# abajcsy/legged_games_gym

Measured on AMD Instinct MI355X. Metric: env-steps/sec (whole node), ANYmal-C flat 4096 envs/GPU, higher is better.
Workload: dtype f32; 1 GPU; anymal_c_flat, 4096 envs/GPU, plane, actuator-net torques, self-collision ON (asset.self_collisions = 0), random-init policy [48, 128, 64, 32, 12] rollout (act = mu + sigma*eps), fixed command (0.5,0,0), obs noise + friction/mass randomisation + pushes on; envs_per_gpu=4096, decimation=4, parallelism=env-sharded x1, state_finite=True, policy=MFMA actor inside k_step (v_mfma_f32_16x16x4_f32, 4 waves)

## Files before the change

legged_games_gym_amd/csrc/lg_device.h:

```cpp
#pragma once
#include <hip/hip_runtime.h>
#include <stdint.h>
#include "../../include/legged_hip.h"

#define LG_DEV __device__ __forceinline__

namespace lg {

struct V3 { float x, y, z; };
LG_DEV V3 v3(float x, float y, float z) { V3 r; r.x = x; r.y = y; r.z = z; return r; }
LG_DEV V3 operator+(V3 a, V3 b) { return v3(a.x + b.x, a.y + b.y, a.z + b.z); }
LG_DEV V3 operator-(V3 a, V3 b) { return v3(a.x - b.x, a.y - b.y, a.z - b.z); }
LG_DEV V3 operator*(V3 a, float s) { return v3(a.x * s, a.y * s, a.z * s); }
LG_DEV float dot(V3 a, V3 b) { return a.x * b.x + a.y * b.y + a.z * b.z; }
LG_DEV V3 cross(V3 a, V3 b) { return v3(a.y * b.z - a.z * b.y, a.z * b.x - a.x * b.z, a.x * b.y - a.y * b.x); }
struct M3 { float m[9]; };
LG_DEV V3 mul(const M3 &R, V3 a) {
    return v3(R.m[0] * a.x + R.m[1] * a.y + R.m[2] * a.z, R.m[3] * a.x + R.m[4] * a.y + R.m[5] * a.z,
              R.m[6] * a.x + R.m[7] * a.y + R.m[8] * a.z);
}
LG_DEV M3 mul(const M3 &A, const M3 &B) {
    M3 C;
#pragma unroll
    for (int i = 0; i < 3; i++)
#pragma unroll
        for (int j = 0; j < 3; j++) C.m[3 * i + j] = A.m[3 * i] * B.m[j] + A.m[3 * i + 1] * B.m[3 + j] + A.m[3 * i + 2] * B.m[6 + j];
    return C;
}
LG_DEV V3 symv(const float *S, V3 a) {
    return v3(S[0] * a.x + S[1] * a.y + S[2] * a.z, S[1] * a.x + S[3] * a.y + S[4] * a.z, S[2] * a.x + S[4] * a.y + S[5] * a.z);
}
struct S6 { V3 w, v; };
LG_DEV S6 operator+(S6 a, S6 b) { S6 r; r.w = a.w + b.w; r.v = a.v + b.v; return r; }
LG_DEV S6 operator*(S6 a, float k) { S6 r; r.w = a.w * k; r.v = a.v * k; return r; }
LG_DEV float dot(S6 a, S6 b) { return dot(a.w, b.w) + dot(a.v, b.v); }

struct AI { float A[6], H[9], M[6]; };
LG_DEV void ai_add(AI &a, const AI &b) {
#pragma unroll
    for (int i = 0; i < 6; i++) { a.A[i] += b.A[i]; a.M[i] += b.M[i]; }
#pragma unroll
    for (int i = 0; i < 9; i++) a.H[i] += b.H[i];
}
LG_DEV void ai_add_point(AI &I, float m, V3 c) {
    float cc = dot(c, c);
    I.A[0] += m * (cc - c.x * c.x); I.A[1] -= m * c.x * c.y; I.A[2] -= m * c.x * c.z;
    I.A[3] += m * (cc - c.y * c.y); I.A[4] -= m * c.y * c.z; I.A[5] += m * (cc - c.z * c.z);
    I.H[1] -= m * c.z; I.H[2] += m * c.y; I.H[3] += m * c.z; I.H[5] -= m * c.x; I.H[6] -= m * c.y; I.H[7] += m * c.x;
    I.M[0] += m; I.M[3] += m; I.M[5] += m;
}
LG_DEV void ai_add_rank1(AI &I, float k, V3 gw, V3 gv) {
    float w[3] = {gw.x, gw.y, gw.z}, v[3] = {gv.x, gv.y, gv.z};
    int t = 0;
#pragma unroll
    for (int i = 0; i < 3; i++)
#pragma unroll
        for (int j = i; j < 3; j++, t++) { I.A[t] += k * w[i] * w[j]; I.M[t] += k * v[i] * v[j]; }
#pragma unroll
    for (int i = 0; i < 3; i++)
#pragma unroll
        for (int j = 0; j < 3; j++) I.H[3 * i + j] += k * w[i] * v[j];
}
LG_DEV S6 ai_mul(const AI &I, S6 s) {
    S6 r;
    M3 H; for (int i = 0; i < 9; i++) H.m[i] = I.H[i];
    r.w = symv(I.A, s.w) + mul(H, s.v);
    r.v = v3(I.H[0] * s.w.x + I.H[3] * s.w.y + I.H[6] * s.w.z, I.H[1] * s.w.x + I.H[4] * s.w.y + I.H[7] * s.w.z,
             I.H[2] * s.w.x + I.H[5] * s.w.y + I.H[8] * s.w.z) + symv(I.M, s.v);
    return r;
}

LG_DEV S6 ai_mul_w(const AI &I, V3 w) {
    S6 r;
    r.w = symv(I.A, w);
    r.v = v3(I.H[0] * w.x + I.H[3] * w.y + I.H[6] * w.z, I.H[1] * w.x + I.H[4] * w.y + I.H[7] * w.z,
             I.H[2] * w.x + I.H[5] * w.y + I.H[8] * w.z);
    return r;
}
LG_DEV void ai_shift(AI &I, S6 &p, V3 d) {
    const int ix[3][3] = {{0, 1, 2}, {1, 3, 4}, {2, 4, 5}};
    float T[9];
#pragma unroll
    for (int j = 0; j < 3; j++) {
        V3 x = cross(d, v3(I.M[ix[0][j]], I.M[ix[1][j]], I.M[ix[2][j]]));
        T[j] = I.H[j] + x.x; T[3 + j] = I.H[3 + j] + x.y; T[6 + j] = I.H[6 + j] + x.z;
    }
    V3 dxh[3], txd[3];
#pragma unroll
    for (int j = 0; j < 3; j++) dxh[j] = cross(d, v3(I.H[3 * j], I.H[3 * j + 1], I.H[3 * j + 2]));
#pragma unroll
    for (int i = 0; i < 3; i++) txd[i] = cross(v3(T[3 * i], T[3 * i + 1], T[3 * i + 2]), d);
    float A2[6];
#pragma unroll
    for (int i = 0; i < 3; i++)
#pragma unroll
        for (int j = i; j < 3; j++) {
            float a = (i == 0) ? dxh[j].x : (i == 1) ? dxh[j].y : dxh[j].z;
            float b = (j == 0) ? txd[i].x : (j == 1) ? txd[i].y : txd[i].z;
            A2[ix[i][j]] = I.A[ix[i][j]] + a - b;
        }
#pragma unroll
    for (int i = 0; i < 6; i++) I.A[i] = A2[i];
#pragma unroll
// ... 187 lines not shown
```

legged_games_gym_amd/csrc/lg_kernels.hip:

```cpp
#include <hip/hip_runtime.h>
#include <math.h>
#include <stdio.h>
#include <string.h>
#include <new>

#define LG_POLICY_BLOCKS_ONLY
#include "lg_host.h"

using namespace lg;

#define LG_BLOCK 64
#define LG_JS 40
#define LG_PASSES 2
#define LG_STEP_WAVES 4

struct AnymalTraits {
    static constexpr int K = 4, L = 3, NREP = 4, NPT = 5;
    static constexpr int pt_joint(int i) { return i < 2 ? 1 : 2; }
    static constexpr int pt_rep(int i) { return i < 2 ? 1 : (i < 4 ? 2 : 3); }
    static constexpr int FOOT_REP = 3;
    static constexpr int NCAP = 3, NGRP = 2;
    static constexpr int cap_p0(int c) { return 2 * c; }
    static constexpr int cap_p1(int c) { return c < 2 ? 2 * c + 1 : 4; }
    static constexpr int cap_grp(int c) { return c == 0 ? 0 : 1; }
// ... 315 lines not shown
        float vn = dot(c.n, c.vc);
        V3 vt = c.vc - c.n * vn;
        V3 f = c.n * (P.contact_stiffness * c.depth - kn * vn) - vt * c.bt + c.fs;
        ai_add_point(IA, dt * c.bt, c.r);
        ai_add_rank1(IA, dt * (kn - c.bt), cross(c.r, c.n), c.n);
        pA.w = pA.w - cross(c.r, f);
        pA.v = pA.v - f;
    }
}
template <bool HF>
LG_DEV void contact_evaluate(Contact &c, const lg_params &P, float kn, float mu, S6 acc, bool more = true) {
    if constexpr (!HF) {
        if (c.on) {
            V3 v1 = c.vc + (acc.v + cross(acc.w, c.r)) * P.sim_dt;
            float fn = plane_normal_force(P, kn, c.depth, v1.z);
            if (fn <= 0.0f) { c.on = false; c.f = v3(0, 0, 0); }
            else {
                c.f = plane_force(c, v1, fn);
                if (!more) return;
                float vtm = plane_slip_speed(v1), cone = mu * fn;
                if (c.bt * vtm > cone) { const float s = -cone / vtm; c.fs = v3(v1.x * s, v1.y * s, 0.0f); c.bt = 0.0f; }
                else if (c.bt > 0.0f) c.bt = fminf(P.friction_damping, cone / fmaxf(vtm, P.stick_velocity));
            }
        }
        return;
    }
    if (c.on) {
        V3 v1 = c.vc + (acc.v + cross(acc.w, c.r)) * P.sim_dt;
        float vn = dot(c.n, v1);
        V3 vt = v1 - c.n * vn;
        float fn = P.contact_stiffness * c.depth - kn * vn;
        if (fn <= 0.0f) { c.on = false; c.f = v3(0, 0, 0); }
        else {
            c.f = c.n * fn - vt * c.bt + c.fs;
            if (!more) return;
            float vtm = sqrtf(dot(vt, vt)), cone = mu * fn;
            if (c.bt * vtm > cone) { c.fs = vt * (-cone / vtm); c.bt = 0.0f; }
            else if (c.bt > 0.0f) c.bt = fminf(P.friction_damping, cone / fmaxf(vtm, P.stick_velocity));
        }
    }
}

LG_DEV float motor_torque(float tau, float qd, float vlim) {
    if (vlim <= 0.0f || tau * qd <= 0.0f) return tau;
    float s = (vlim - fabsf(qd)) / (0.1f * vlim);
    return tau * fminf(fmaxf(s, 0.0f), 1.0f);
}
LG_DEV V3 clamp_norm(V3 a, float lim) {
    float n2 = dot(a, a);
    if (!(n2 <= lim * lim)) { float k = (n2 > 0.0f && n2 < INFINITY) ? lim * __builtin_amdgcn_rsqf(n2) : 0.0f; return a * k; }
    return a;
}

LG_DEV void body_terms(V3 grav, float m, V3 com_l, const float *Il, const M3 &R, V3 w, V3 v, AI &I0, S6 &p0) {
    V3 c = mul(R, com_l);
    M3 Ilf; Ilf.m[0] = Il[0]; Ilf.m[1] = Il[1]; Ilf.m[2] = Il[2]; Ilf.m[3] = Il[1]; Ilf.m[4] = Il[3]; Ilf.m[5] = Il[4];
    Ilf.m[6] = Il[2]; Ilf.m[7] = Il[4]; Ilf.m[8] = Il[5];
    M3 Rt;
#pragma unroll
    for (int i = 0; i < 3; i++)
#pragma unroll
        for (int j2 = 0; j2 < 3; j2++) Rt.m[3 * i + j2] = R.m[3 * j2 + i];
    M3 Ic = mul(mul(R, Ilf), Rt);
#pragma unroll
    for (int i = 0; i < 9; i++) I0.H[i] = 0.0f;
#pragma unroll
    for (int i = 0; i < 6; i++) I0.M[i] = 0.0f;
    I0.A[0] = Ic.m[0]; I0.A[1] = Ic.m[1]; I0.A[2] = Ic.m[2]; I0.A[3] = Ic.m[4]; I0.A[4] = Ic.m[5]; I0.A[5] = Ic.m[8];
    ai_add_point(I0, m, c);
    V3 l = (v + cross(w, c)) * m;
    V3 n = mul(Ic, w) + cross(c, l);
    V3 fg = grav * m;
    p0.w = (cross(w, n) + cross(v, l)) - cross(c, fg);
    p0.v = cross(w, l) - fg;
}
struct FkOut { M3 R; V3 db, ax, w, v; };
LG_DEV FkOut fk_joint(const float *tj, const M3 &Rpar, V3 wpar, V3 vpar, float q, float qd) {
    FkOut o;
    o.db = mul(Rpar, v3(tj[J_POS], tj[J_POS + 1], tj[J_POS + 2]));
    M3 Rfix;
#pragma unroll
    for (int i = 0; i < 9; i++) Rfix.m[i] = tj[J_ROT + i];
    const M3 Rz = mul(Rpar, Rfix);
    o.ax = v3(Rz.m[0], Rz.m[3], Rz.m[6]);
    float sn, cs;
    __sincosf(q, &sn, &cs);
#pragma unroll
    for (int r = 0; r < 3; r++) {
        o.R.m[3 * r] = Rz.m[3 * r];
        o.R.m[3 * r + 1] = cs * Rz.m[3 * r + 1] + sn * Rz.m[3 * r + 2];
        o.R.m[3 * r + 2] = cs * Rz.m[3 * r + 2] - sn * Rz.m[3 * r + 1];
    }
    o.w = wpar + o.ax * qd;
    o.v = vpar + cross(wpar, o.db);
    return o;
}
#define LG_BT_QUADS 7
LG_DEV void bt_store(float4 (*dst)[LG_BLOCK], int lane, const AI &I, const S6 &p) {
    dst[0][lane] = make_float4(I.A[0], I.A[1], I.A[2], I.A[3]); dst[1][lane] = make_float4(I.A[4], I.A[5], I.H[0], I.H[1]);
    dst[2][lane] = make_float4(I.H[2], I.H[3], I.H[4], I.H[5]); dst[3][lane] = make_float4(I.H[6], I.H[7], I.H[8], I.M[0]);
    dst[4][lane] = make_float4(I.M[1], I.M[2], I.M[3], I.M[4]); dst[5][lane] = make_float4(I.M[5], p.w.x, p.w.y, p.w.z);
    dst[6][lane] = make_float4(p.v.x, p.v.y, p.v.z, 0.0f);
}
LG_DEV void bt_load(const float4 (*src)[LG_BLOCK], int lane, AI &I, S6 &p) {
    float4 a = src[0][lane], b = src[1][lane], c = src[2][lane], d = src[3][lane], e = src[4][lane], f = src[5][lane], g = src[6][lane];
    I.A[0] = a.x; I.A[1] = a.y; I.A[2] = a.z; I.A[3] = a.w; I.A[4] = b.x; I.A[5] = b.y; I.H[0] = b.z; I.H[1] = b.w;
    I.H[2] = c.x; I.H[3] = c.y; I.H[4] = c.z; I.H[5] = c.w; I.H[6] = d.x; I.H[7] = d.y; I.H[8] = d.z; I.M[0] = d.w;
    I.M[1] = e.x; I.M[2] = e.y; I.M[3] = e.z; I.M[4] = e.w; I.M[5] = f.x; p.w = v3(f.y, f.z, f.w); p.v = v3(g.x, g.y, g.z);
}

#define LG_SC_REC 4
template <class T> struct SelfLds {
    float4 pos[T::NPT][LG_BLOCK];
    float4 vel[T::NPT][LG_BLOCK];
    float4 grp[T::NGRP][LG_BLOCK];
    float4 basepose[5][LG_BLOCK];
    float4 rec[T::K][T::NGRP][LG_SC_REC][LG_BLOCK];
    alignas(16) int ready[LG_STEP_WAVES];
    float4 base_pts[LG_MAX_BASE_POINTS];
};
LG_DEV V3 xyz(float4 a) { return v3(a.x, a.y, a.z); }
template <bool SA, bool SB> LG_DEV void seg_seg_closest(V3 a0, V3 a1, V3 b0, V3 b1, float &s, float &t) {
    const float eps = 1e-12f;
    V3 d1 = a1 - a0, d2 = b1 - b0, r = a0 - b0;
    float a = SA ? 0.0f : dot(d1, d1), e = SB ? 0.0f : dot(d2, d2), f = SB ? 0.0f : dot(d2, r);
    if ((SA || a <= eps) && (SB || e <= eps)) { s = 0.0f; t = 0.0f; }
    else if (SA || a <= eps) { s = 0.0f; t = fminf(fmaxf(f / e, 0.0f), 1.0f); }
    else {
        float c = dot(d1, r);
        if (SB || e <= eps) { t = 0.0f; s = fminf(fmaxf(-c / a, 0.0f), 1.0f); }
        else {
            float b = dot(d1, d2), denom = a * e - b * b;
            s = (denom > eps) ? fminf(fmaxf((b * f - c * e) / denom, 0.0f), 1.0f) : 0.0f;
            t = (b * s + f) / e;
            if (t < 0.0f) { t = 0.0f; s = fminf(fmaxf(-c / a, 0.0f), 1.0f); }
            else if (t > 1.0f) { t = 1.0f; s = fminf(fmaxf((b - c) / a, 0.0f), 1.0f); }
        }
    }
}
struct SelfHit { V3 n, pa, pb; float depth, f0; };
template <bool SA, bool SB, class Vel>
LG_DEV bool capsule_contact(const lg_params &P, float kn, V3 a0, V3 a1, float ra, V3 b0, V3 b1, float rb, Vel vel, SelfHit &h) {
    float s, t;
    seg_seg_closest<SA, SB>(a0, a1, b0, b1, s, t);
    V3 ca = a0 + (a1 - a0) * s, cb = b0 + (b1 - b0) * t, diff = ca - cb;
    float dist = sqrtf(dot(diff, diff));
    float d = ra + rb - dist;
    if (!(d > -P.contact_margin)) return false;
    V3 va0, va1, vb0, vb1;
    vel(va0, va1, vb0, vb1);
    h.n = diff * (1.0f / fmaxf(dist, 1e-9f));
    V3 va = va0 + (va1 - va0) * s, vb = vb0 + (vb1 - vb0) * t;
    float f = P.contact_stiffness * d - kn * dot(h.n, va - vb);
    if (!(d > 0.0f || f > 0.0f)) return false;
    h.depth = d; h.f0 = fmaxf(f, 0.0f); h.pa = ca - h.n * ra; h.pb = cb + h.n * rb;
    return true;
}
template <class T>
LG_DEV void self_detect(const KArgs &A, const float *lds_tab, int ln, int m, SelfLds<T> &sc) {
    constexpr int K = T::K, NCAP = T::NCAP, NGRP = T::NGRP;
    const lg_params &P = A.P;
// ... 47 lines not shown
#pragma unroll
    for (int ga = 0; ga < NGRP; ga++) {
        SelfHit best; best.depth = -1e30f; best.f0 = 0.0f; best.n = best.pa = best.pb = v3(0, 0, 0);
        float best_mB = 1.0f; int best_i = 0;
        const unsigned gbits = ((1u << NGRP) - 1u) << (ga * NGRP);
        if (any && __builtin_amdgcn_ballot_w64((cand & gbits) != 0) != 0) {
#pragma unroll 1
            for (int i = T::grp_cap_lo(ga); i < T::grp_cap_hi(ga); i++) {
                const int ip0 = T::cap_p0(i), ip1 = T::cap_p1(i);
                const float4 pa0 = sc.pos[ip0][ln], pa1 = sc.pos[ip1][ln];
                const bool sa = ip0 == ip1;
                const int nother = m == 0 ? nbc : NCAP;
#pragma unroll 1
                for (int j = 0; j < nother; j++) {
                    const unsigned bit = 1u << (ga * NGRP + (m == 0 ? 0 : T::cap_grp(j)));
                    if (__builtin_amdgcn_ballot_w64((cand & bit) != 0) == 0) continue;
                    SelfHit h; bool hit = false; float mB;
                    if (m == 0) {
                        const V3 e0 = base_end(j, 0), e1 = base_end(j, 1);
                        auto vel = [&](V3 &va0, V3 &va1, V3 &vb0, V3 &vb1) {
                            va0 = xyz(sc.vel[ip0][ln]); va1 = xyz(sc.vel[ip1][ln]); vb0 = v0 + cross(w0, e0); vb1 = v0 + cross(w0, e1);
                        };
                        mB = A.base.mass_robot;
                        if (cand & bit) hit = sa ? capsule_contact<true, false>(P, kn, xyz(pa0), xyz(pa1), pa0.w, e0, e1, sc.base_pts[2 * j].w, vel, h)
                                                 : capsule_contact<false, false>(P, kn, xyz(pa0), xyz(pa1), pa0.w, e0, e1, sc.base_pts[2 * j].w, vel, h);
                    } else {
                        const int jp0 = T::cap_p0(j), jp1 = T::cap_p1(j);
                        const float4 pb0 = sc.pos[jp0][lp], pb1 = sc.pos[jp1][lp];
                        const bool sb = jp0 == jp1;
                        auto vel = [&](V3 &va0, V3 &va1, V3 &vb0, V3 &vb1) {
                            va0 = xyz(sc.vel[ip0][ln]); va1 = xyz(sc.vel[ip1][ln]); vb0 = xyz(sc.vel[jp0][lp]); vb1 = xyz(sc.vel[jp1][lp]);
                        };
                        mB = tabp[T::pt_joint(jp0) * LG_JS + J_SUBM];
                        if (cand & bit) {
                            if (sa && sb) hit = capsule_contact<true, true>(P, kn, xyz(pa0), xyz(pa1), pa0.w, xyz(pb0), xyz(pb1), pb0.w, vel, h);
                            else if (sa) hit = capsule_contact<true, false>(P, kn, xyz(pa0), xyz(pa1), pa0.w, xyz(pb0), xyz(pb1), pb0.w, vel, h);
                            else if (sb) hit = capsule_contact<false, true>(P, kn, xyz(pa0), xyz(pa1), pa0.w, xyz(pb0), xyz(pb1), pb0.w, vel, h);
                            else hit = capsule_contact<false, false>(P, kn, xyz(pa0), xyz(pa1), pa0.w, xyz(pb0), xyz(pb1), pb0.w, vel, h);
                        }
                    }
                    if (hit && h.depth > best.depth) { best = h; best_mB = mB; best_i = i; }
                }
            }
        }
        const bool on = best.depth > -1e29f;
        const float mA = tab[T::pt_joint(T::grp_c0(ga)) * LG_JS + J_SUBM];
        sc.rec[m][ga][0][ln] = make_float4(best.n.x, best.n.y, best.n.z, best.f0);
        sc.rec[m][ga][1][ln] = make_float4(best.pa.x, best.pa.y, best.pa.z, on ? dt * kn * (1.0f + mA / best_mB) : -1.0f);
        sc.rec[m][ga][2][ln] = make_float4(best.pb.x, best.pb.y, best.pb.z, on ? dt * kn * (1.0f + best_mB / mA) : -1.0f);
        sc.rec[m][ga][3][ln] = make_float4(best.f0 / (1.0f + kn * dt * (1.0f / mA + 1.0f / best_mB)), (float)best_i, 0.0f, 0.0f);
    }
}
template <class T>
LG_DEV bool self_apply(int ln, const V3 (&db)[T::L], AI (&I0)[T::L], S6 (&p0)[T::L], const SelfLds<T> &sc) {
    float coef[T::K][T::NGRP];
    unsigned mask = 0;
#pragma unroll
    for (int m = 0; m < T::K; m++)
#pragma unroll
        for (int g = 0; g < T::NGRP; g++) coef[m][g] = sc.rec[m][g][1][ln].w;
#pragma unroll
    for (int m = 0; m < T::K; m++)
#pragma unroll
        for (int g = 0; g < T::NGRP; g++) if (coef[m][g] >= 0.0f) mask |= 1u << (m * T::NGRP + g);
    if (__builtin_amdgcn_ballot_w64(mask != 0) == 0) return false;
#pragma unroll
    for (int m = 0; m < T::K; m++) {
#pragma unroll
        for (int g = 0; g < T::NGRP; g++) {
            const int jc = T::pt_joint(T::grp_c0(g));
            const bool hit = (mask >> (m * T::NGRP + g)) & 1u;
            if (__builtin_amdgcn_ballot_w64(hit) == 0) continue;
            if (hit) {
                const float4 r0 = sc.rec[m][g][0][ln], r1 = sc.rec[m][g][1][ln];
                V3 rj = db[0];
#pragma unroll
                for (int jj = 1; jj <= jc; jj++) rj = rj + db[jj];
                const V3 n = xyz(r0), r = xyz(r1) - rj, f = n * r0.w;
                ai_add_rank1(I0[jc], r1.w, cross(r, n), n);
                p0[jc].w = p0[jc].w - cross(r, f); p0[jc].v = p0[jc].v - f;
            }
        }
    }
    return true;
}

struct NoWait { LG_DEV void operator()() const {} };
template <class T, bool HF, class Ready = NoWait, bool OFFLOAD = false, bool SC = false, bool LAST_LEAN = false, bool ROLL = false>
LG_DEV void physics_substep(const KArgs &A, const float *tab, int lane_k, float (&root)[13], float (&q)[T::L], float (&qd)[T::L],
                            const float (&tau)[T::L], float base_mass, float mu,
                            float (&Frep)[T::NREP][3], float (&Fbase)[3], Ready torques_ready = Ready(),
                            const float4 (*bt)[LG_BT_QUADS][LG_BLOCK] = nullptr, float4 (*fkout)[4][LG_BLOCK] = nullptr,
                            volatile int *fk_ready = nullptr, int substep_no = 0, SelfLds<T> *sc = nullptr, bool last = true,
                            bool sc_on_helpers = false ) {
    constexpr int K = T::K, L = T::L, NPT = T::NPT;
    const lg_params &P = A.P;
    const float dt = P.sim_dt;
    const int spin_limit_early = ROLL ? A.spin_limit : 0;
    const V3 grav = v3(P.gravity[0], P.gravity[1], P.gravity[2]);
    const float kn = P.contact_stiffness * dt + P.contact_damping;

    const M3 R0 = quat_to_mat(root + 3);
    const V3 w0 = v3(root[10], root[11], root[12]), v0 = v3(root[7], root[8], root[9]);
    V3 db[L], ax[L];
    S6 C[L];
    AI I0[L], I0b;
    S6 p0[L], p0b;
    Contact cb, cl[NPT];
    HfFetch fb, fl[NPT];
    V3 sgc[T::NGRP];
    {
        float bm = base_mass;
        if (L > 3) asm volatile("" : "+v"(bm));
        float mass_scale = bm / A.base.mass, Il[6];
#pragma unroll
        for (int i = 0; i < 6; i++) Il[i] = A.base.inertia[i] * mass_scale;
        body_terms(grav, bm, v3(A.base.com[0], A.base.com[1], A.base.com[2]), Il, R0, w0, v0, I0b, p0b);
        static_assert(K <= LG_MAX_BASE_POINTS, "one base point per lane at most");
        {
            const float bp[4] = {tab[Tab<T>::BPT], tab[Tab<T>::BPT + 1], tab[Tab<T>::BPT + 2], tab[Tab<T>::BPT + 3]};
            cb.r = mul(R0, v3(bp[0], bp[1], bp[2]));
            cb.vc = v0 + cross(w0, cb.r);
            cb.depth = bp[3];
            fb = hf_fetch<HF>(A, root[0] + cb.r.x, root[1] + cb.r.y);
        }
    }
    {
        M3 Rpar = R0;
        V3 rpar = v3(0, 0, 0), wpar = w0, vpar = v0;
#pragma unroll
        for (int j = 0; j < L; j++) {
            const float *tj = tab + j * LG_JS;
            const FkOut fk = fk_joint(tj, Rpar, wpar, vpar, q[j], qd[j]);
            db[j] = fk.db; ax[j] = fk.ax;
            const V3 rj = rpar + db[j];
            const M3 &Rj = fk.R;
            const V3 wj = fk.w, vj = fk.v;
            C[j].w = cross(wj, ax[j]) * qd[j];
            C[j].v = cross(vj, ax[j]) * qd[j];
            if (!OFFLOAD) {
                float Il[6];
#pragma unroll
                for (int i = 0; i < 6; i++) Il[i] = tj[J_INERTIA + i];
                body_terms(grav, tj[J_MASS], v3(tj[J_COM], tj[J_COM + 1], tj[J_COM + 2]), Il, Rj, wj, vj, I0[j], p0[j]);
            } else {
                const int ln = threadIdx.x % LG_BLOCK;
                fkout[j][0][ln] = make_float4(Rj.m[0], Rj.m[1], Rj.m[2], Rj.m[3]);
                fkout[j][1][ln] = make_float4(Rj.m[4], Rj.m[5], Rj.m[6], Rj.m[7]);
                fkout[j][2][ln] = make_float4(Rj.m[8], wj.x, wj.y, wj.z);
                fkout[j][3][ln] = make_float4(vj.x, vj.y, vj.z, 0.0f);
                if (j == L - 1) {
                    asm volatile("s_waitcnt lgkmcnt(0)" ::: "memory");
                    if (ln == 0 && A.debug_skip != 1) *fk_ready = substep_no;
                }
            }
#pragma unroll
            for (int i = 0; i < NPT; i++) if (T::pt_joint(i) == j) {
                const float *tp = tab + L * LG_JS + 4 * i;
                cl[i].r = mul(Rj, v3(tp[0], tp[1], tp[2]));
                V3 pw = rj + cl[i].r;
                cl[i].vc = vj + cross(wj, cl[i].r);
                cl[i].depth = tp[3];
                cl[i].vtn = root[2] + pw.z;
                fl[i] = hf_fetch<HF>(A, root[0] + pw.x, root[1] + pw.y);
                if (SC) {
                    const int ln = threadIdx.x % LG_BLOCK;
                    sc->pos[i][ln] = make_float4(pw.x, pw.y, pw.z, tp[3]);
                    sc->vel[i][ln] = make_float4(cl[i].vc.x, cl[i].vc.y, cl[i].vc.z, 0.0f);
#pragma unroll
                    for (int g = 0; g < T::NGRP; g++) {
                        if (T::grp_c0(g) == i) sgc[g] = pw;
                        if (T::grp_c1(g) == i) sgc[g] = (sgc[g] + pw) * 0.5f;
                    }
                }
            }
            Rpar = Rj; rpar = rj; wpar = wj; vpar = vj;
        }
    }
    {
        float dep; V3 n;
        hf_contact<HF>(A, fb, root[2] + cb.r.z, cb.depth, dep, n);
        contact_setup<HF>(cb, P, mu, cb.r, n, dep, cb.vc, v3(Fbase[0], Fbase[1], Fbase[2]));
        cb.on = cb.on && (lane_k < A.base.num_pts);
#pragma unroll
        for (int i = 0; i < NPT; i++) {
            hf_contact<HF>(A, fl[i], cl[i].vtn, cl[i].depth, dep, n);
            contact_setup<HF>(cl[i], P, mu, cl[i].r, n, dep, cl[i].vc,
                          v3(Frep[T::pt_rep(i)][0], Frep[T::pt_rep(i)][1], Frep[T::pt_rep(i)][2]));
        }
    }

    if constexpr (SC) {
        const int ln = threadIdx.x % LG_BLOCK;
#pragma unroll
        for (int g = 0; g < T::NGRP; g++) sc->grp[g][ln] = make_float4(sgc[g].x, sgc[g].y, sgc[g].z, tab[Tab<T>::GRP + g]);
        sc->basepose[0][ln] = make_float4(R0.m[0], R0.m[1], R0.m[2], 0.0f); sc->basepose[1][ln] = make_float4(R0.m[3], R0.m[4], R0.m[5], 0.0f);
        sc->basepose[2][ln] = make_float4(R0.m[6], R0.m[7], R0.m[8], 0.0f);
        sc->basepose[3][ln] = make_float4(w0.x, w0.y, w0.z, 0.0f); sc->basepose[4][ln] = make_float4(v0.x, v0.y, v0.z, 0.0f);
    }
    LG_PROF(PF_KINEMATICS);
    torques_ready();
    if (OFFLOAD) {
#pragma unroll
        for (int j = 0; j < L; j++) bt_load(bt[j], threadIdx.x % LG_BLOCK, I0[j], p0[j]);
    }
    bool any_self = false;
    bool sc_missed = false;
    LG_PROF(PF_TORQUE);
    S6 U[L], acc0;
    float Dinv[L], uu[L], vl[L];
#pragma unroll
    for (int j = 0; j < L; j++) vl[j] = 0.0f;
#pragma unroll 1
    for (int pass = 0; pass < LG_PASSES; pass++) {
        const bool more = !LAST_LEAN || pass < LG_PASSES - 1;
        AI Ia; S6 pa;
        if constexpr (SC) if (pass == LG_PASSES - 1) {
            const int ln = threadIdx.x % LG_BLOCK;
            if (sc_on_helpers) {
                volatile int4 *rdy = reinterpret_cast<volatile int4 *>(sc->ready);
                bool arrived = false;
                for (int spin = 0; spin < (ROLL ? spin_limit_early : A.spin_limit); spin++) {
                    const int r1 = rdy->y, r2 = rdy->z, r3 = rdy->w;
                    if (min(r1, min(r2, r3)) >= substep_no) { arrived = true; break; }
                    __builtin_amdgcn_s_sleep(1);
                }
                sc_missed |= !arrived;
                __builtin_amdgcn_wave_barrier();
            } else {
                __builtin_amdgcn_wave_barrier();
#pragma unroll 1
                for (int m = 0; m < K; m++) self_detect<T>(A, tab - lane_k * Tab<T>::STRIDE, ln, m, *sc);
                __builtin_amdgcn_wave_barrier();
            }
            any_self = self_apply<T>(ln, db, I0, p0, *sc);
        }
#pragma unroll
        for (int j = L - 1; j >= 0; j--) {
            const float *tj = tab + j * LG_JS;
            AI IA = I0[j]; S6 pA = p0[j];
#pragma unroll
            for (int i = 0; i < NPT; i++) if (T::pt_joint(i) == j) { LG_PROF_COUNT(0, cl[i].on); contact_assemble<HF>(cl[i], P, kn, IA, pA); }
            if (j < L - 1) { ai_add(IA, Ia); pA = pA + pa; }
            U[j] = ai_mul_w(IA, ax[j]);
            float damp = tj[J_DAMP];
            float D = dot(ax[j], U[j].w) + tj[J_ARM] + dt * damp;
            float u = motor_torque(tau[j], qd[j], tj[J_VLIM]) - dot(ax[j], pA.w) - damp * qd[j];
            float lo = tj[J_LO], hi = tj[J_HI];
            LG_PROF_COUNT(3, lo <= hi && (q[j] + dt * qd[j] < lo || q[j] + dt * qd[j] > hi));
            LG_PROF_COUNT(4, vl[j] != 0.0f);
            if (lo <= hi) {
                float qp = q[j] + dt * qd[j];
                bool blo = qp < lo, bhi = qp > hi;
                if (blo || bhi) {
                    float viol = q[j] - (blo ? lo : hi);
                    float kl = P.limit_stiffness * dt + P.limit_damping;
                    D += dt * kl;
                    u += -P.limit_stiffness * viol - kl * qd[j];
                }
            }
            if (vl[j] != 0.0f) {
                float Bv = 100.0f * D / dt;
                u += -Bv * (qd[j] - vl[j] * tj[J_VLIM]);
                D += dt * Bv;
            }
            Dinv[j] = __builtin_amdgcn_rcpf(D); uu[j] = u;
            Ia = IA;
            ai_add_rank1(Ia, -Dinv[j], U[j].w, U[j].v);
            pa = (pA + ai_mul(Ia, C[j])) + U[j] * (u * Dinv[j]);
            ai_shift(Ia, pa, db[j]);
        }
        LG_PROF(PF_INWARD);
        LG_PROF_COUNT(1, cb.on);
        LG_PROF_COUNT(2, any_self);
        contact_assemble<HF>(cb, P, kn, Ia, pa);
        if (SC && any_self) {
            const int ln = threadIdx.x % LG_BLOCK;
#pragma unroll
            for (int g = 0; g < T::NGRP; g++) {
                const float4 r2 = sc->rec[0][g][2][ln];
                if (r2.w >= 0.0f) {
                    const float4 r0 = sc->rec[0][g][0][ln];
                    const V3 n = xyz(r0), cxn = cross(xyz(r2), n);
                    ai_add_rank1(Ia, r2.w, cxn, n);
                    pa.w = pa.w + cxn * r0.w; pa.v = pa.v + n * r0.w;
                }
            }
        }
        group_sum<K>(Ia, pa);
        AI IAb = I0b; S6 pAb = p0b;
        ai_add(IAb, Ia); pAb = pAb + pa;
        float rhs[6] = {-pAb.w.x, -pAb.w.y, -pAb.w.z, -pAb.v.x, -pAb.v.y, -pAb.v.z}, a0[6];
        bool ok = solve6(IAb, rhs, a0);
        if (!ok) { a0[0] = a0[1] = a0[2] = a0[3] = a0[4] = a0[5] = 0.0f; }
        acc0.w = v3(a0[0], a0[1], a0[2]); acc0.v = v3(a0[3], a0[4], a0[5]);
        contact_evaluate<HF>(cb, P, kn, mu, acc0, more);
        LG_PROF(PF_BASE);
        S6 a = acc0;
#pragma unroll
        for (int j = 0; j < L; j++) {
            S6 ap;
            ap.w = a.w + C[j].w;
            ap.v = (a.v + cross(a.w, db[j])) + C[j].v;
            float qdd = (uu[j] - dot(U[j], ap)) * Dinv[j];
            a.w = ap.w + ax[j] * qdd;
            a.v = ap.v;
            uu[j] = qdd;
            if (more) {
                float lim = tab[j * LG_JS + J_VLIM], qn = qd[j] + dt * qdd;
                if (lim > 0.0f && vl[j] == 0.0f && fabsf(qn) > lim) vl[j] = qn > 0.0f ? 1.0f : -1.0f;
            }
#pragma unroll
            for (int i = 0; i < NPT; i++) if (T::pt_joint(i) == j) contact_evaluate<HF>(cl[i], P, kn, mu, a, more);
        }
        LG_PROF(PF_OUTWARD);
    }

    if constexpr (SC) if (sc_missed && threadIdx.x % LG_BLOCK == 0) lg_report(A.status, LG_STATUS_SELF_COLLISION_TIMEOUT);
#pragma unroll
    for (int j = 0; j < L; j++) {
        float v = qd[j] + dt * uu[j];
        float lim = tab[j * LG_JS + J_VLIM];
        if (lim > 0.0f) v = fminf(fmaxf(v, -lim), lim);
        qd[j] = v;
        q[j] += dt * v;
    }
    {
        V3 a_lin = acc0.v + cross(w0, v0);
        V3 w1 = clamp_norm(w0 + acc0.w * dt, 1000.0f), v1 = clamp_norm(v0 + a_lin * dt, 1000.0f);
        root[7] = v1.x; root[8] = v1.y; root[9] = v1.z; root[10] = w1.x; root[11] = w1.y; root[12] = w1.z;
        root[0] += dt * v1.x; root[1] += dt * v1.y; root[2] += dt * v1.z;
        float x = root[3], y = root[4], z = root[5], w = root[6], hx = 0.5f * dt * w1.x, hy = 0.5f * dt * w1.y, hz = 0.5f * dt * w1.z;
        float nx = x + (hx * w + hy * z - hz * y), ny = y + (hy * w + hz * x - hx * z), nz = z + (hz * w + hx * y - hy * x);
        float nw = w - (hx * x + hy * y + hz * z);
        float inv = 1.0f / sqrtf(nx * nx + ny * ny + nz * nz + nw * nw);
        root[3] = nx * inv; root[4] = ny * inv; root[5] = nz * inv; root[6] = nw * inv;
    }
#pragma unroll
    for (int r = 0; r < T::NREP; r++) {
        V3 f = v3(0, 0, 0);
#pragma unroll
        for (int i = 0; i < NPT; i++) if (T::pt_rep(i) == r) f = f + cl[i].f;
        Frep[r][0] = f.x; Frep[r][1] = f.y; Frep[r][2] = f.z;
// ... 356 lines not shown
    if (levels && t == 0) {
        float acc = 0.0f;
        for (int w = 0; w < (int)(blockDim.x >> 6); w++) acc += level_part[w];
        A.B.episode_means[R] = acc / (float)P.num_envs;
    }
}
LG_DEV void roll_finish(const KArgs &A, int t, int64_t step0, int rt0, int rt1) {
    const lg_params &P = A.P;
    const int R = P.num_reward_slots, stride = LG_NUM_REWARD_TERMS + 2;
    int last = -1;
    for (int s = rt1 - 1; s >= rt0 && last < 0; s--)
        if (__hip_atomic_load(A.roll.extras + (size_t)s * stride + R, __ATOMIC_RELAXED, __HIP_MEMORY_SCOPE_AGENT) > 0.0f) last = s;
    if (last >= 0 && t < R) {
        const float v = __hip_atomic_load(A.roll.extras + (size_t)last * stride + t, __ATOMIC_RELAXED, __HIP_MEMORY_SCOPE_AGENT);
        const float c = __hip_atomic_load(A.roll.extras + (size_t)last * stride + R, __ATOMIC_RELAXED, __HIP_MEMORY_SCOPE_AGENT);
        A.B.episode_means[t] = v / c / P.max_episode_length_s;
    }
    if (t == 0 && A.B.step_counter) A.B.step_counter[0] = step0 + rt1 - 1;
    if (t == 0 && A.roll.cursor) A.roll.cursor[0] = rt1;
    __builtin_amdgcn_s_waitcnt(0);
    __builtin_amdgcn_wave_barrier();
    for (int i = rt0 * stride + t; i < rt1 * stride; i += 64) __hip_atomic_store(A.roll.extras + i, 0.0f, __ATOMIC_RELAXED, __HIP_MEMORY_SCOPE_AGENT);
}

LG_DEV void redraw_reset_command(const KArgs &A, float x0, float x1, int e, int64_t step, float *obs_row) {
    const lg_params &P = A.P; const lg_buffers &B = A.B;
    float u[4], cmd[4];
#pragma unroll
    for (int i = 0; i < 4; i++) cmd[i] = B.commands[(size_t)e * 4 + i];
    rand4(P.seed, e, step, RNG_CMD_RESET, 0, u);
    resample_commands_x(P, x0, x1, u, cmd);
#pragma unroll
    for (int i = 0; i < 4; i++) B.commands[(size_t)e * 4 + i] = cmd[i];
    const float c = P.clip_observations;
    obs_row[9] = fminf(fmaxf(cmd[0] * P.obs_scale_lin_vel, -c), c); obs_row[10] = fminf(fmaxf(cmd[1] * P.obs_scale_lin_vel, -c), c);
    obs_row[11] = fminf(fmaxf(cmd[2] * P.obs_scale_ang_vel, -c), c);
}
LG_DEV void curriculum_apply(const KArgs &A, int t, int nt, int64_t step, float cnt, const uint8_t *resets, float *obs) {
    const lg_params &P = A.P;
    if (!(cnt > 0.0f) || P.cmd_curriculum_slot < 0) return;
    double *xr = A.B.cmd_range;
    const double mean_sum = (double)A.B.episode_means[P.cmd_curriculum_slot] * P.cmd_episode_length_s;
    const double lo0 = xr[0], hi0 = xr[1];
    if (!(mean_sum / P.cmd_max_episode_length > 0.8 * P.cmd_tracking_scale_dt)) return;
    const double lo = fmin(fmax(lo0 - 0.5, -P.cmd_max_curriculum), 0.0), hi = fmin(fmax(hi0 + 0.5, 0.0), P.cmd_max_curriculum);
    if (lo == lo0 && hi == hi0) return;
    __syncthreads();
    if (t == 0) { xr[0] = lo; xr[1] = hi; }
    const float x0 = (float)lo, x1 = (float)hi;
    for (int e = t; e < P.num_envs; e += nt)
        if (resets[e]) redraw_reset_command(A, x0, x1, e, step, obs + (size_t)e * P.num_obs);
}

template <bool OFF, int L = 3> struct StepSharedT {
    float pose[LG_BLOCK][5];
    float hsum[LG_STEP_WAVES][LG_BLOCK];
    float root_z[LG_BLOCK];
    int   rst[LG_BLOCK];
    float r_t[LG_NUM_REWARD_TERMS][LG_BLOCK];
    float4 fk[OFF ? L : 1][4][LG_BLOCK];
    float4 bt[OFF ? L : 1][LG_BT_QUADS][LG_BLOCK];
    int    fk_ready;
};

struct EpisodeSums {
    float sum[LG_NUM_REWARD_TERMS] = {};
    LG_DEV void load(const KArgs &A, int e) {
#pragma unroll
        for (int t = 0; t < LG_NUM_REWARD_TERMS; t++) {
            const int slot = A.P.reward_slot[t];
            sum[t] = slot >= 0 ? A.B.episode_sums[(size_t)slot * A.P.num_envs + e] : 0.0f;
        }
    }
    template <int K, class SH> LG_DEV void update(const KArgs &A, int e, int lane, SH &sh, bool keep, float *accum) {
        const lg_params &P = A.P;
        const bool reset = keep && sh.rst[lane] != 0;
        if (keep) {
#pragma unroll
            for (int t = 0; t < LG_NUM_REWARD_TERMS; t++) {
                const int slot = P.reward_slot[t];
                if (slot >= 0) {
                    sum[t] += sh.r_t[t][lane];
                    A.B.episode_sums[(size_t)slot * P.num_envs + e] = reset ? 0.0f : sum[t];
                }
            }
        }
        const unsigned long long finished = __ballot(reset);
        if (finished == 0) return;
#pragma unroll
        for (int t = 0; t < LG_NUM_REWARD_TERMS; t++) sh.r_t[t][lane] = reset ? sum[t] : 0.0f;
        __builtin_amdgcn_fence(__ATOMIC_RELEASE, "wavefront");
        __builtin_amdgcn_wave_barrier();
        if (lane < LG_NUM_REWARD_TERMS) {
            int slot = -1;
#pragma unroll
            for (int t = 0; t < LG_NUM_REWARD_TERMS; t++) slot = lane == t ? P.reward_slot[t] : slot;
            float tot = 0.0f;
            for (int i = 0; i < LG_BLOCK; i += K) tot += sh.r_t[lane][i];
            if (slot >= 0) atomicAdd(accum + slot, tot);
        } else if (lane == LG_NUM_REWARD_TERMS) atomicAdd(accum + P.num_reward_slots, (float)__popcll(finished));
    }
};

template <class T, bool NET, bool HF, int NW, bool SC = false> struct HelperWave {
    static constexpr bool OFF = NW >= 2;
    static LG_DEV void run(const KArgs &A, int wave, int lane, int e, int k, int d0, bool live, int64_t step, const float *tab,
                           float2 (*lds_x)[LG_BLOCK], float (*lds_tau)[LG_BLOCK], StepSharedT<OFF, T::L> &sh, SelfLds<T> *sc = nullptr,
                           const float *lds_tab = nullptr, ResetRand<T> *reset_rand = nullptr, int *s_last = nullptr, float4 (*hnoise)[LG_BLOCK] = nullptr,
                           int sub0 = 0 , float *roll_accum = nullptr ,
                           bool tick_step = false ) {
        const lg_buffers &B = A.B;
        const lg_params &P = A.P;
        const int j = wave - 1;
        bool missed = false;
        LstmSplit st;
        float (*part[4])[4] = {st.h0, st.c0, st.h1, st.c1};
        float *row[4] = {nullptr, nullptr, nullptr, nullptr};
        LstmLane LW;
        if (NET) {
            const size_t plane = (size_t)P.num_envs * (T::K * T::L);
            LW = lstm_load(A.weights, lane);
            row[0] = B.sea_hidden_state + (size_t)(d0 + j) * 8; row[1] = B.sea_cell_state + (size_t)(d0 + j) * 8;
            row[2] = B.sea_hidden_state + (plane + d0 + j) * 8; row[3] = B.sea_cell_state + (plane + d0 + j) * 8;
#pragma unroll
            for (int a = 0; a < 4; a++) {
                float4 lo = reinterpret_cast<const float4 *>(row[a])[0], hi = reinterpret_cast<const float4 *>(row[a])[1];
                float u[8] = {lo.x, lo.y, lo.z, lo.w, hi.x, hi.y, hi.z, hi.w};
                lstm_split(u, part[a][0], part[a][1]);
            }
        }
        if (NET || OFF) {
            for (int it = 0; it < P.decimation; it++) {
                __syncthreads();
                float tau_j = 0.0f;
                if (NET) {
                    const float2 x = lds_x[j][lane];
                    tau_j = actuator_step_mfma(LW, x.x, x.y, st);
                    lds_tau[j][lane] = tau_j;
                }
                if (OFF) {
                    volatile int *flag = &sh.fk_ready;
                    int spin = 0;
                    for (; *flag < sub0 + it + 1 && spin < A.spin_limit; spin++) __builtin_amdgcn_s_sleep(1);
                    missed |= spin >= A.spin_limit;
#pragma unroll 1
                    for (int b = j; b < T::L; b += NW - 1) {
                        const float4 f0 = sh.fk[b][0][lane], f1 = sh.fk[b][1][lane], f2 = sh.fk[b][2][lane], f3 = sh.fk[b][3][lane];
                        M3 R; R.m[0] = f0.x; R.m[1] = f0.y; R.m[2] = f0.z; R.m[3] = f0.w; R.m[4] = f1.x; R.m[5] = f1.y; R.m[6] = f1.z; R.m[7] = f1.w; R.m[8] = f2.x;
                        const float *tb = tab + b * LG_JS;
                        float Il[6];
#pragma unroll
                        for (int i = 0; i < 6; i++) Il[i] = tb[J_INERTIA + i];
                        AI I0; S6 p0;
                        body_terms(v3(P.gravity[0], P.gravity[1], P.gravity[2]), tb[J_MASS], v3(tb[J_COM], tb[J_COM + 1], tb[J_COM + 2]), Il, R,
                                   v3(f2.y, f2.z, f2.w), v3(f3.x, f3.y, f3.z), I0, p0);
                        bt_store(sh.bt[b], lane, I0, p0);
                    }
                }
                __syncthreads();
                if constexpr (SC && NW == LG_STEP_WAVES) {
                    self_detect<T>(A, lds_tab, lane, wave, *sc);
                    if (wave == LG_STEP_WAVES - 1) self_detect<T>(A, lds_tab, lane, 0, *sc);
                    asm volatile("s_waitcnt lgkmcnt(0)" ::: "memory");
                    if (lane == 0 && A.debug_skip != 2) sc->ready[wave] = sub0 + it + 1;
                }
            }
        }
        reset_rand->draw(P, e, k, step, lane, wave - 1, NW - 1);
        if (P.measure_heights && P.add_noise) {
            const int nchunk = (P.num_height_points + 3) >> 2;
#pragma unroll
            for (int b = 0; b < HeightCrew<T, NW>::NCH; b++) {
                const int c = k + b * HeightCrew<T, NW>::NV;
                if (b % (NW > 1 ? NW - 1 : 1) == wave - 1 && c < nchunk) {
                    float r[4];
                    rand4(P.seed, e, step, RNG_NOISE_H, c, r);
                    hnoise[b][lane] = make_float4(r[0], r[1], r[2], r[3]);
                }
            }
        }
        if (NET) {
#pragma unroll
            for (int a = 0; a < 4; a++) {
                float u[8];
                lstm_unsplit(part[a][0], part[a][1], u);
                if (live) {
                    reinterpret_cast<float4 *>(row[a])[0] = make_float4(u[0], u[1], u[2], u[3]);
                    reinterpret_cast<float4 *>(row[a])[1] = make_float4(u[4], u[5], u[6], u[7]);
                }
            }
        }
        __syncthreads();
        HeightCrew<T, NW> hc;
        float hs = 0.0f;
        if (P.measure_heights) hs = hc.template sample<HF>(A, e, k + T::K * wave, live, sh.pose[lane][0], sh.pose[lane][1], sh.pose[lane][2], sh.pose[lane][3], sh.pose[lane][4]);
        sh.hsum[wave][lane] = hs;
        __syncthreads();
        const bool keeper = wave == 1 && live && k == 0;
        EpisodeSums es;
        if (keeper) es.load(A, e);
        float un[HeightCrew<T, NW>::NCH][4];
        if (P.measure_heights) hc.draw_noise(P, e, k + T::K * wave, step, un);
        __syncthreads();
        if (wave == 1) {
            es.template update<T::K>(A, e, lane, sh, keeper, roll_accum ? roll_accum : accum_slot(A, step));
            if (roll_accum) {  }
// ... 2 lines not shown
                int lv = keeper ? __hip_atomic_load(A.B.terrain_levels + e, __ATOMIC_RELAXED, __HIP_MEMORY_SCOPE_AGENT) : 0;
#pragma unroll
                for (int o = 32; o > 0; o >>= 1) lv += __shfl_xor(lv, o);
                if (lane == 0) __hip_atomic_store(level_parts_slot(A, step, gridDim.x) + blockIdx.x, lv, __ATOMIC_RELAXED, __HIP_MEMORY_SCOPE_AGENT);
            }
            if (tick_step) {  }
            else if (A.defer) {
                if (lane == 0 && atomicAdd(A.done_counter, 1u) == gridDim.x - 1) {
                    if (B.step_counter) B.step_counter[0] = step;
                    __hip_atomic_store(A.done_counter, 0u, __ATOMIC_RELAXED, __HIP_MEMORY_SCOPE_AGENT);
                }
            } else {
            asm volatile("s_waitcnt vmcnt(0)" ::: "memory");
            if (lane == 0) {
                const unsigned int ticket = atomicAdd(A.done_counter, 1u);
                const int last = ticket == gridDim.x - 1;
                if (last) __hip_atomic_store(A.done_counter, 0u, __ATOMIC_RELAXED, __HIP_MEMORY_SCOPE_AGENT);
                *s_last = last;
            }
            }
            }
        }
        if (P.measure_heights) hc.write_obs(A, e, k + T::K * wave, live, step, sh.root_z[lane], un);
        if (missed && lane == 0) lg_report(A.status, LG_STATUS_FRAME_HANDOVER_TIMEOUT);
        if (NET) {
            const bool reset = sh.rst[lane] != 0 && live;
            if (__ballot(reset) != 0 && reset) {
#pragma unroll
                for (int a = 0; a < 4; a++) {
                    reinterpret_cast<float4 *>(row[a])[0] = make_float4(0.0f, 0.0f, 0.0f, 0.0f);
                    reinterpret_cast<float4 *>(row[a])[1] = make_float4(0.0f, 0.0f, 0.0f, 0.0f);
                }
            }
        }
    }
};

template <bool SC, class T> struct SelfStore { char unused; LG_DEV SelfLds<T> *get() { return nullptr; } };
template <class T> struct SelfStore<true, T> { SelfLds<T> lds; LG_DEV SelfLds<T> *get() { return &lds; } };

template <class T, bool NET, bool HF, bool POL = false, int NW = LG_STEP_WAVES, bool SC = false, bool ROLL = false>
__global__ void __launch_bounds__(NW * LG_BLOCK) k_step(const KArgs A_launch) {
    const KArgs &A = A_launch;
    static_assert(!NET || (NW == LG_STEP_WAVES && 1 + T::L == NW), "one actuator wave per joint of the limb");
    static_assert(!ROLL || (POL && !HF), "the multi-step rollout kernel is the fused-actor kernel on the plane");
    static_assert(!POL || (NET && NW == LG_POLICY_WAVES && T::K * T::L <= 16), "fused policy needs the four-wave actuator-net kernel");
    constexpr int K = T::K, L = T::L, ND = K * L, NREP = T::NREP;
    const lg_params &P = A.P;
    const lg_buffers &B = A.B;
    __shared__ float lds_tab[T::K * Tab<T>::STRIDE];
    __shared__ float2 lds_x[NET ? L : 1][LG_BLOCK];
    __shared__ float lds_tau[NET ? L : 1][LG_BLOCK];
    constexpr bool OFF = NW >= 2;
    __shared__ StepSharedT<OFF, L> sh;
    __shared__ SelfStore<SC, T> sc_store;
    __shared__ ResetRand<T> reset_rand;
    __shared__ float4 hnoise[NW > 1 ? HeightCrew<T, NW>::NCH : 1][LG_BLOCK];
    __shared__ int s_last;
    __shared__ float4 pol_xa[POL ? 4 : 1][64], pol_xb[POL ? 8 : 1][64], pol_xy[1][64];
    __shared__ float lds_act[POL ? 16 : 1][16];
    __shared__ float lds_obs[ROLL ? 16 : 1][48];
    __shared__ float s_tick_cnt;
    __shared__ float s_xr[2];
    __shared__ int s_roll[2];
    int roll_begin = 0;
    if (ROLL && A.P.cmd_curriculum && A.roll.sub > 0) {
        roll_begin = A.roll.cursor[0];
        if (roll_begin >= A.roll.steps) return;
    }
    LG_PROF_BEGIN();
    if (threadIdx.x == 0) sh.fk_ready = 0;
    if constexpr (SC) {
        if (threadIdx.x < LG_STEP_WAVES) sc_store.get()->ready[threadIdx.x] = 0;
        stage_base_points<T>(A, sc_store.get());
    }
    stage_limb_table<T>(A, lds_tab);

    const int N = P.num_envs;
    const int wave = threadIdx.x / LG_BLOCK, lane = threadIdx.x % LG_BLOCK;
    const int tid = blockIdx.x * LG_BLOCK + lane;
    int e = tid / K;
    const int k = tid % K;
    const bool live = e < N;
    if (!live) e = N - 1;
    const float *tab = lds_tab + k * Tab<T>::STRIDE;
    const int d0 = e * ND + k * L;
    const int64_t step0 = A.step >= 0 ? A.step : B.step_counter[0] + 1 - roll_begin;
    if (threadIdx.x == 0) {
        cmd_x_range_f32(A, s_xr);
        if (ROLL) {
            int roll_end = A.roll.steps;
            if (P.cmd_curriculum) {
                const int64_t M = P.max_episode_length, first = step0 + roll_begin;
                roll_end = min(roll_end, roll_begin + (int)((M - first % M) % M) + 1);
            }
            s_roll[0] = roll_begin; s_roll[1] = roll_end;
        }
    }
    const int e_wg = e, k_wg = k;
    auto one_step = [&](const int rt) {
    const KArgs &A = step_args<ROLL>(A_launch);
    const lg_params &P = A.P;
    const lg_buffers &B = A.B;
    const int N = P.num_envs;
    int tix = threadIdx.x;
    if constexpr (ROLL) asm volatile("" : "+v"(tix));
    const int wave = tix / LG_BLOCK, lane = tix % LG_BLOCK;
// ... 1140 lines not shown
```

Measured before the change: 76.07 million env-steps/s.

## Store compact rigid-body inertia in LDS and fold self-contacts per joint

On the non-heightfield path, the per-body spatial inertia passed from helper waves to the physics wave is packed compactly (6 rotational terms, mass-times-COM vector, mass) instead of the full 21-float articulated inertia. This cuts the LDS handoff from 7 to 4 float4s per body and lowers register pressure. Self-collision contributions are no longer applied to all link inertias up front. A hit mask is computed instead, and each joint folds its own contacts while the backward pass expands its inertia. The cost is extra expansion arithmetic per joint and more template branching.

```diff
diff --git a/legged_games_gym_amd/csrc/lg_device.h b/legged_games_gym_amd/csrc/lg_device.h
--- a/legged_games_gym_amd/csrc/lg_device.h
+++ b/legged_games_gym_amd/csrc/lg_device.h
@@ -49,6 +49,14 @@
     I.H[1] -= m * c.z; I.H[2] += m * c.y; I.H[3] += m * c.z; I.H[5] -= m * c.x; I.H[6] -= m * c.y; I.H[7] += m * c.x;
     I.M[0] += m; I.M[3] += m; I.M[5] += m;
 }
+struct RI { float A[6]; V3 h; float m; };
+LG_DEV void ri_expand(AI &I, const RI &r) {
+#pragma unroll
+    for (int i = 0; i < 6; i++) I.A[i] = r.A[i];
+    I.H[0] = 0.0f; I.H[1] = -r.h.z; I.H[2] = r.h.y; I.H[3] = r.h.z; I.H[4] = 0.0f; I.H[5] = -r.h.x; I.H[6] = -r.h.y; I.H[7] = r.h.x; I.H[8] = 0.0f;
+    I.M[0] = r.m; I.M[1] = 0.0f; I.M[2] = 0.0f; I.M[3] = r.m; I.M[4] = 0.0f; I.M[5] = r.m;
+}
+LG_DEV void ri_expand(AI &I, const AI &r) { I = r; }
 LG_DEV void ai_add_rank1(AI &I, float k, V3 gw, V3 gv) {
     float w[3] = {gw.x, gw.y, gw.z}, v[3] = {gv.x, gv.y, gv.z};
     int t = 0;
diff --git a/legged_games_gym_amd/csrc/lg_kernels.hip b/legged_games_gym_amd/csrc/lg_kernels.hip
--- a/legged_games_gym_amd/csrc/lg_kernels.hip
+++ b/legged_games_gym_amd/csrc/lg_kernels.hip
@@ -391,6 +391,30 @@
     return a;
 }
 
+LG_DEV void body_terms(V3 grav, float m, V3 com_l, const float *Il, const M3 &R, V3 w, V3 v, RI &I0, S6 &p0) {
+    V3 c = mul(R, com_l);
+    M3 Ilf; Ilf.m[0] = Il[0]; Ilf.m[1] = Il[1]; Ilf.m[2] = Il[2]; Ilf.m[3] = Il[1]; Ilf.m[4] = Il[3]; Ilf.m[5] = Il[4];
+    Ilf.m[6] = Il[2]; Ilf.m[7] = Il[4]; Ilf.m[8] = Il[5];
+    M3 Rt;
+#pragma unroll
+    for (int i = 0; i < 3; i++)
+#pragma unroll
+        for (int j2 = 0; j2 < 3; j2++) Rt.m[3 * i + j2] = R.m[3 * j2 + i];
+    M3 Ic = mul(mul(R, Ilf), Rt);
+    I0.A[0] = Ic.m[0]; I0.A[1] = Ic.m[1]; I0.A[2] = Ic.m[2]; I0.A[3] = Ic.m[4]; I0.A[4] = Ic.m[5]; I0.A[5] = Ic.m[8];
+    {
+        float cc = dot(c, c);
+        I0.A[0] += m * (cc - c.x * c.x); I0.A[1] -= m * c.x * c.y; I0.A[2] -= m * c.x * c.z;
+        I0.A[3] += m * (cc - c.y * c.y); I0.A[4] -= m * c.y * c.z; I0.A[5] += m * (cc - c.z * c.z);
+    }
+    I0.h = v3(prod_rn(m, c.x), prod_rn(m, c.y), prod_rn(m, c.z));
+    I0.m = m;
+    V3 l = (v + cross(w, c)) * m;
+    V3 n = mul(Ic, w) + cross(c, l);
+    V3 fg = grav * m;
+    p0.w = (cross(w, n) + cross(v, l)) - cross(c, fg);
+    p0.v = cross(w, l) - fg;
+}
 LG_DEV void body_terms(V3 grav, float m, V3 com_l, const float *Il, const M3 &R, V3 w, V3 v, AI &I0, S6 &p0) {
     V3 c = mul(R, com_l);
     M3 Ilf; Ilf.m[0] = Il[0]; Ilf.m[1] = Il[1]; Ilf.m[2] = Il[2]; Ilf.m[3] = Il[1]; Ilf.m[4] = Il[3]; Ilf.m[5] = Il[4];
@@ -434,7 +458,13 @@
     o.v = vpar + cross(wpar, o.db);
     return o;
 }
-#define LG_BT_QUADS 7
+template <bool HF> struct RigidOf { typedef RI type; };
+template <> struct RigidOf<true> { typedef AI type; };
+template <bool HF> struct BtQuads { static constexpr int N = HF ? 7 : 4; };
+LG_DEV void bt_store(float4 (*dst)[LG_BLOCK], int lane, const RI &I, const S6 &p) {
+    dst[0][lane] = make_float4(I.A[0], I.A[1], I.A[2], I.A[3]); dst[1][lane] = make_float4(I.A[4], I.A[5], I.h.x, I.h.y);
+    dst[2][lane] = make_float4(I.h.z, I.m, p.w.x, p.w.y); dst[3][lane] = make_float4(p.w.z, p.v.x, p.v.y, p.v.z);
+}
 LG_DEV void bt_store(float4 (*dst)[LG_BLOCK], int lane, const AI &I, const S6 &p) {
     dst[0][lane] = make_float4(I.A[0], I.A[1], I.A[2], I.A[3]); dst[1][lane] = make_float4(I.A[4], I.A[5], I.H[0], I.H[1]);
     dst[2][lane] = make_float4(I.H[2], I.H[3], I.H[4], I.H[5]); dst[3][lane] = make_float4(I.H[6], I.H[7], I.H[8], I.M[0]);
@@ -446,6 +476,11 @@
     I.A[0] = a.x; I.A[1] = a.y; I.A[2] = a.z; I.A[3] = a.w; I.A[4] = b.x; I.A[5] = b.y; I.H[0] = b.z; I.H[1] = b.w;
     I.H[2] = c.x; I.H[3] = c.y; I.H[4] = c.z; I.H[5] = c.w; I.H[6] = d.x; I.H[7] = d.y; I.H[8] = d.z; I.M[0] = d.w;
     I.M[1] = e.x; I.M[2] = e.y; I.M[3] = e.z; I.M[4] = e.w; I.M[5] = f.x; p.w = v3(f.y, f.z, f.w); p.v = v3(g.x, g.y, g.z);
+}
+LG_DEV void bt_load(const float4 (*src)[LG_BLOCK], int lane, RI &I, S6 &p) {
+    float4 a = src[0][lane], b = src[1][lane], c = src[2][lane], d = src[3][lane];
+    I.A[0] = a.x; I.A[1] = a.y; I.A[2] = a.z; I.A[3] = a.w; I.A[4] = b.x; I.A[5] = b.y; I.h = v3(b.z, b.w, c.x); I.m = c.y;
+    p.w = v3(c.z, c.w, d.x); p.v = v3(d.y, d.z, d.w);
 }
 
 #define LG_SC_REC 4
@@ -599,6 +634,20 @@
     }
 }
 template <class T>
+LG_DEV bool self_mask(int ln, const SelfLds<T> &sc, unsigned &mask) {
+    float coef[T::K][T::NGRP];
+    mask = 0;
+#pragma unroll
+    for (int m = 0; m < T::K; m++)
+#pragma unroll
+        for (int g = 0; g < T::NGRP; g++) coef[m][g] = sc.rec[m][g][1][ln].w;
+#pragma unroll
+    for (int m = 0; m < T::K; m++)
+#pragma unroll
+        for (int g = 0; g < T::NGRP; g++) if (coef[m][g] >= 0.0f) mask |= 1u << (m * T::NGRP + g);
+    return __builtin_amdgcn_ballot_w64(mask != 0) != 0;
+}
+template <class T>
 LG_DEV bool self_apply(int ln, const V3 (&db)[T::L], AI (&I0)[T::L], S6 (&p0)[T::L], const SelfLds<T> &sc) {
     float coef[T::K][T::NGRP];
     unsigned mask = 0;
@@ -632,12 +681,35 @@
     return true;
 }
 
+template <class T>
+LG_DEV void self_fold(int j, unsigned mask, int ln, const V3 (&db)[T::L], AI &IA, S6 &pA, const SelfLds<T> &sc) {
+#pragma unroll
+    for (int m = 0; m < T::K; m++) {
+#pragma unroll
+        for (int g = 0; g < T::NGRP; g++) {
+            const int jc = T::pt_joint(T::grp_c0(g));
+            if (jc != j) continue;
+            const bool hit = (mask >> (m * T::NGRP + g)) & 1u;
+            if (__builtin_amdgcn_ballot_w64(hit) == 0) continue;
+            if (hit) {
+                const float4 r0 = sc.rec[m][g][0][ln], r1 = sc.rec[m][g][1][ln];
+                V3 rj = db[0];
+#pragma unroll
+                for (int jj = 1; jj <= jc; jj++) rj = rj + db[jj];
+                const V3 n = xyz(r0), r = xyz(r1) - rj, f = n * r0.w;
+                ai_add_rank1(IA, r1.w, cross(r, n), n);
+                pA.w = pA.w - cross(r, f); pA.v = pA.v - f;
+            }
+        }
+    }
+}
+
 struct NoWait { LG_DEV void operator()() const {} };
 template <class T, bool HF, class Ready = NoWait, bool OFFLOAD = false, bool SC = false, bool LAST_LEAN = false, bool ROLL = false>
 LG_DEV void physics_substep(const KArgs &A, const float *tab, int lane_k, float (&root)[13], float (&q)[T::L], float (&qd)[T::L],
                             const float (&tau)[T::L], float base_mass, float mu,
                             float (&Frep)[T::NREP][3], float (&Fbase)[3], Ready torques_ready = Ready(),
-                            const float4 (*bt)[LG_BT_QUADS][LG_BLOCK] = nullptr, float4 (*fkout)[4][LG_BLOCK] = nullptr,
+                            const float4 (*bt)[BtQuads<HF>::N][LG_BLOCK] = nullptr, float4 (*fkout)[4][LG_BLOCK] = nullptr,
                             volatile int *fk_ready = nullptr, int substep_no = 0, SelfLds<T> *sc = nullptr, bool last = true,
                             bool sc_on_helpers = false ) {
     constexpr int K = T::K, L = T::L, NPT = T::NPT;
@@ -651,7 +723,7 @@
     const V3 w0 = v3(root[10], root[11], root[12]), v0 = v3(root[7], root[8], root[9]);
     V3 db[L], ax[L];
     S6 C[L];
-    AI I0[L], I0b;
+    typename RigidOf<HF>::type I0[L], I0b;
     S6 p0[L], p0b;
     Contact cb, cl[NPT];
     HfFetch fb, fl[NPT];
@@ -752,6 +824,8 @@
         for (int j = 0; j < L; j++) bt_load(bt[j], threadIdx.x % LG_BLOCK, I0[j], p0[j]);
     }
     bool any_self = false;
+    const int ln_sc = threadIdx.x % LG_BLOCK;
+    unsigned self_hits = 0;
     bool sc_missed = false;
     LG_PROF(PF_TORQUE);
     S6 U[L], acc0;
@@ -780,12 +854,15 @@
                 for (int m = 0; m < K; m++) self_detect<T>(A, tab - lane_k * Tab<T>::STRIDE, ln, m, *sc);
                 __builtin_amdgcn_wave_barrier();
             }
-            any_self = self_apply<T>(ln, db, I0, p0, *sc);
+            if constexpr (HF) any_self = self_apply<T>(ln, db, I0, p0, *sc);
+            else any_self = self_mask<T>(ln, *sc, self_hits);
         }
 #pragma unroll
         for (int j = L - 1; j >= 0; j--) {
             const float *tj = tab + j * LG_JS;
-            AI IA = I0[j]; S6 pA = p0[j];
+            AI IA; S6 pA = p0[j];
+            ri_expand(IA, I0[j]);
+            if (SC && !HF && any_self) self_fold<T>(j, self_hits, ln_sc, db, IA, pA, *sc);
 #pragma unroll
             for (int i = 0; i < NPT; i++) if (T::pt_joint(i) == j) { LG_PROF_COUNT(0, cl[i].on); contact_assemble<HF>(cl[i], P, kn, IA, pA); }
             if (j < L - 1) { ai_add(IA, Ia); pA = pA + pa; }
@@ -835,7 +912,8 @@
             }
         }
         group_sum<K>(Ia, pa);
-        AI IAb = I0b; S6 pAb = p0b;
+        AI IAb; S6 pAb = p0b;
+        ri_expand(IAb, I0b);
         ai_add(IAb, Ia); pAb = pAb + pa;
         float rhs[6] = {-pAb.w.x, -pAb.w.y, -pAb.w.z, -pAb.v.x, -pAb.v.y, -pAb.v.z}, a0[6];
         bool ok = solve6(IAb, rhs, a0);
@@ -1298,14 +1376,14 @@
         if (resets[e]) redraw_reset_command(A, x0, x1, e, step, obs + (size_t)e * P.num_obs);
 }
 
-template <bool OFF, int L = 3> struct StepSharedT {
+template <bool OFF, int L = 3, bool HF = false> struct StepSharedT {
     float pose[LG_BLOCK][5];
     float hsum[LG_STEP_WAVES][LG_BLOCK];
     float root_z[LG_BLOCK];
     int   rst[LG_BLOCK];
     float r_t[LG_NUM_REWARD_TERMS][LG_BLOCK];
     float4 fk[OFF ? L : 1][4][LG_BLOCK];
-    float4 bt[OFF ? L : 1][LG_BT_QUADS][LG_BLOCK];
+    float4 bt[OFF ? L : 1][BtQuads<HF>::N][LG_BLOCK];
     int    fk_ready;
 };
 
@@ -1351,7 +1429,7 @@
 template <class T, bool NET, bool HF, int NW, bool SC = false> struct HelperWave {
     static constexpr bool OFF = NW >= 2;
     static LG_DEV void run(const KArgs &A, int wave, int lane, int e, int k, int d0, bool live, int64_t step, const float *tab,
-                           float2 (*lds_x)[LG_BLOCK], float (*lds_tau)[LG_BLOCK], StepSharedT<OFF, T::L> &sh, SelfLds<T> *sc = nullptr,
+                           float2 (*lds_x)[LG_BLOCK], float (*lds_tau)[LG_BLOCK], StepSharedT<OFF, T::L, HF> &sh, SelfLds<T> *sc = nullptr,
                            const float *lds_tab = nullptr, ResetRand<T> *reset_rand = nullptr, int *s_last = nullptr, float4 (*hnoise)[LG_BLOCK] = nullptr,
                            int sub0 = 0 , float *roll_accum = nullptr ,
                            bool tick_step = false ) {
@@ -1397,7 +1475,7 @@
                         float Il[6];
 #pragma unroll
                         for (int i = 0; i < 6; i++) Il[i] = tb[J_INERTIA + i];
-                        AI I0; S6 p0;
+                        typename RigidOf<HF>::type I0; S6 p0;
                         body_terms(v3(P.gravity[0], P.gravity[1], P.gravity[2]), tb[J_MASS], v3(tb[J_COM], tb[J_COM + 1], tb[J_COM + 2]), Il, R,
                                    v3(f2.y, f2.z, f2.w), v3(f3.x, f3.y, f3.z), I0, p0);
                         bt_store(sh.bt[b], lane, I0, p0);
@@ -1506,7 +1584,7 @@
     __shared__ float2 lds_x[NET ? L : 1][LG_BLOCK];
     __shared__ float lds_tau[NET ? L : 1][LG_BLOCK];
     constexpr bool OFF = NW >= 2;
-    __shared__ StepSharedT<OFF, L> sh;
+    __shared__ StepSharedT<OFF, L, HF> sh;
     __shared__ SelfStore<SC, T> sc_store;
     __shared__ ResetRand<T> reset_rand;
     __shared__ float4 hnoise[NW > 1 ? HeightCrew<T, NW>::NCH : 1][LG_BLOCK];
```

Result: faster. 76.95 million env-steps/s (median of 6 runs) (+1.2%).
